# aniketntnu/WordDiffusion

Measured on AMD Instinct MI355X. Metric: denoised 64x256 word images/sec (1000-step DDPM), whole job, higher is better.
Workload: dtype bf16x3

## Files before the change

### include/wdiff_hip.h

```cpp
#ifndef WDIFF_HIP_H
#define WDIFF_HIP_H

#include <stdint.h>

#ifdef __cplusplus
extern "C" {
#endif

#define WD_OK 0
#define WD_EINVAL (-1)
#define WD_ELAUNCH (-2)
#define WD_ESTATE (-3)

#define WD_ACT_NONE 0
#define WD_ACT_SILU 1
#define WD_ACT_GEGLU 2

typedef uint16_t wd_bf16;

#define WD_MAX_KSPLIT 64

typedef struct wd_src {
    const wd_bf16* hi;
    const wd_bf16* lo;
// ... 76 lines not shown
    int32_t resid_ld;
    float* out_f32;
    int32_t out_ld;
    wd_bf16* out_hi;
    wd_bf16* out_lo;
    int32_t out_pl_ld;
    const wd_bf16* w3_hi;
    const wd_bf16* w3_lo;
    const float* b3;
    const float* resid3;
    int32_t resid3_ld;
    double* stat_part;
    int32_t stat_cpg;
    int32_t hw_out;
    int32_t npass;
} wd_ff_args;
int wd_ff_fused(const wd_ff_args* args, void* stream);
int wd_ff_supported(int c, int inner);
int wd_ff_args_bytes(void);

int wd_gemm_auto_ksplit(int m, int n, int ktot, int64_t ws_floats);
int wd_gemm_args_bytes(void);
int wd_gemm_experimental(void);

int wd_gn_nchunk(int hw);
int wd_gn_stats(const float* x, int ld, int batch, int hw, int c, int cpg, double* part, void* stream);
int wd_gn_fold_chunks(const double* part, int batch, int nchunk, int ngroups, double* out, void* stream);

int wd_gn_apply(const float* x, int ld, int batch, int hw, int c, int cpg, const double* part, int nchunk, int part_cpg,
                const float* gamma, const float* beta, float eps, int silu,
// ... 204 lines not shown
```

### worddiffusion_amd/_native.py

```python
from __future__ import annotations

import ctypes as C
import os
import re

_HERE = os.path.dirname(os.path.abspath(__file__))
LIB_PATH = os.environ.get("WDIFF_LIB") or os.path.join(_HERE, "libwdiff_hip.so")
HEADER_PATH = os.path.join(os.path.dirname(_HERE), "include", "wdiff_hip.h")

WD_OK, WD_EINVAL, WD_ELAUNCH, WD_ESTATE = 0, -1, -2, -3
ACT_NONE, ACT_SILU, ACT_GEGLU = 0, 1, 2
NCLASS = 13
CLASS_NAMES = ("gemm", "gn_stats", "gn_apply", "layernorm", "attention", "other", "gemm_other_tiles", "gemm_splitk_reduce",
               "gemm_two_per_cu", "gemm_weights_to_registers", "feed_forward_fused", "weight_gradient", "gemm_small_maps_whole_k")

_vp = C.c_void_p
_i = C.c_int
_f = C.c_float
_u64 = C.c_uint64


class WdSrc(C.Structure):
    _fields_ = [("hi", _vp), ("lo", _vp), ("gather", _vp), ("ld", C.c_int32), ("c", C.c_int32),
                ("ntaps", C.c_int32), ("hw_src", C.c_int32)]
# ... 7 lines not shown
                ("out_hi", _vp), ("out_lo", _vp), ("out_pl_ld", C.c_int32), ("tile", C.c_int32),
                ("w_layout", C.c_int32), ("slab_rows", C.c_int32), ("ksplit", C.c_int32), ("ws", _vp),
                ("ws_floats", C.c_int64), ("stat_part", _vp), ("stat_cpg", C.c_int32), ("dbg", C.c_int32),
                ("tickets", _vp), ("ntickets", C.c_int32), ("gn_gamma", _vp), ("gn_beta", _vp), ("gn_eps", C.c_float),
                ("gn_silu", C.c_int32), ("gn_cpg", C.c_int32), ("a32", _vp), ("a32_ld", C.c_int32), ("a32_part", _vp),
                ("a32_nchunk", C.c_int32), ("a32_pcpg", C.c_int32), ("a32_cpg", C.c_int32), ("a32_gamma", _vp), ("a32_beta", _vp),
                ("a32_eps", C.c_float), ("a32_silu", C.c_int32), ("ln_gamma", _vp), ("ln_beta", _vp), ("ln_eps", C.c_float),
                ("w_ngroups", C.c_int32), ("w_group_stride", C.c_int64)]


class WdFfArgs(C.Structure):
    _fields_ = [("x_hi", _vp), ("x_lo", _vp), ("x_ld", C.c_int32), ("m", C.c_int32), ("c", C.c_int32), ("inner", C.c_int32),
                ("w1_hi", _vp), ("w1_lo", _vp), ("b1", _vp), ("w2_hi", _vp), ("w2_lo", _vp), ("b2", _vp), ("resid", _vp),
                ("resid_ld", C.c_int32), ("out_f32", _vp), ("out_ld", C.c_int32), ("out_hi", _vp), ("out_lo", _vp),
                ("out_pl_ld", C.c_int32), ("w3_hi", _vp), ("w3_lo", _vp), ("b3", _vp), ("resid3", _vp), ("resid3_ld", C.c_int32),
                ("stat_part", _vp), ("stat_cpg", C.c_int32), ("hw_out", C.c_int32), ("npass", C.c_int32)]


class WdDwArgs(C.Structure):
    _fields_ = [("d_hi", _vp), ("d_lo", _vp), ("x_hi", _vp), ("x_lo", _vp), ("gather", _vp), ("grad", _vp), ("ws", _vp),
                ("ws_floats", C.c_int64), ("d_ld", C.c_int32), ("x_ld", C.c_int32), ("grad_ld", C.c_int32), ("ntaps", C.c_int32),
                ("hw_out", C.c_int32), ("hw_src", C.c_int32), ("m", C.c_int32), ("n", C.c_int32), ("c", C.c_int32),
                ("npass", C.c_int32), ("accumulate", C.c_int32), ("nslice", C.c_int32), ("dbg", C.c_int32), ("reserved", C.c_int32),
                ("stamps", _vp), ("items", _vp), ("nitems", C.c_int32), ("reserved2", C.c_int32)]


class WdDwItem(C.Structure):
    _fields_ = [("d_hi", _vp), ("d_lo", _vp), ("x_hi", _vp), ("x_lo", _vp), ("grad", _vp), ("d_ld", C.c_int32), ("x_ld", C.c_int32),
                ("grad_ld", C.c_int32), ("accumulate", C.c_int32)]


# ... 144 lines not shown
```

### worddiffusion_amd/csrc/wd_ff.hip

```cpp
#include "wd_gemm_epi.h"

namespace {

constexpr int FNT = 512;
constexpr int FBM = 64;
constexpr int FC = 320;
constexpr int FCH = 128;
constexpr int FRING = 6;
constexpr int F_MAX_INNER = 2048;
constexpr int FGRP = 30;
constexpr uint32_t F_OOB = 0x80000000u;

typedef __attribute__((ext_vector_type(4))) unsigned f_u32x4;

__device__ __forceinline__ int f_lds_off(int row, int ch) { return row * 128 + ((ch ^ ((row >> 1) & 7)) << 4); }

template <int NPASS, bool PROJ>
__global__ void __launch_bounds__(FNT, 1) wd_ff_kernel(const wd_ff_args a) {
#if defined(__HIP_DEVICE_COMPILE__)
    constexpr int NPL = (NPASS == 1) ? 1 : 2;
    constexpr int SLAB = 2 * FBM * 128;
    constexpr int A_BYTES = 5 * SLAB;
    constexpr int H_BYTES = 2 * SLAB;
    extern __shared__ __attribute__((aligned(16))) char smem[];
    char* s_a = smem;
    char* s_h = smem + A_BYTES;
    float* s_b1 = reinterpret_cast<float*>(smem + A_BYTES + 2 * H_BYTES);

    const int m0 = blockIdx.x * FBM;
    const int tid = threadIdx.x;
    const int lane = tid & 63;
    const int wave = __builtin_amdgcn_readfirstlane(tid >> 6);
    const int kh = wave >> 2, cg = wave & 3;
    const int l15 = lane & 15, lq = lane >> 4;
// ... 22 lines not shown
                ring[slot][p] = __builtin_bit_cast(bf16x8, __builtin_amdgcn_raw_buffer_load_b128(srd, lane16, so, 0));
            }
        } else if (g < 20) {
            const uint32_t so = (uint32_t)(((g >> 1) * nct1 + 2 * (j * 8 + wave) + (g & 1)) * 1024);
#pragma unroll
            for (int p = 0; p < NPL; ++p)
                ring[slot][p] = __builtin_bit_cast(bf16x8, __builtin_amdgcn_raw_buffer_load_b128(p ? srd1_lo : srd1_hi, vo, live ? so : 0u, 0));
        } else {
            const int q = (g - 20) / 5, t = (g - 20) % 5;
            const uint32_t so = (uint32_t)(((4 * j + 2 * kh + q) * (FC / 16) + 5 * cg + t) * 1024);
#pragma unroll
            for (int p = 0; p < NPL; ++p)
                ring[slot][p] = __builtin_bit_cast(bf16x8, __builtin_amdgcn_raw_buffer_load_b128(p ? srd2_lo : srd2_hi, vo, live ? so : 0u, 0));
        }
    };
#pragma unroll
    for (int g = 0; g < FRING; ++g) issue(g, g, 0);

    {
        const __amdgpu_buffer_rsrc_t sx_hi = make_srd(a.x_hi), sx_lo = make_srd(a.x_lo ? a.x_lo : a.x_hi);
        const int arow = tid >> 3, ach = tid & 7;
        const uint32_t vo = (m0 + arow < a.m) ? (uint32_t)(m0 + arow) * (uint32_t)(a.x_ld * 2) + (uint32_t)(ach * 16) : F_OOB;
        f_u32x4 v[5][NPL];
#pragma unroll
        for (int sl = 0; sl < 5; ++sl)
#pragma unroll
            for (int p = 0; p < NPL; ++p) v[sl][p] = __builtin_amdgcn_raw_buffer_load_b128(p ? sx_lo : sx_hi, vo, sl * 128, 0);
        const int dst = f_lds_off(arow, ach);
#pragma unroll
        for (int sl = 0; sl < 5; ++sl)
#pragma unroll
            for (int p = 0; p < NPL; ++p) *reinterpret_cast<f_u32x4*>(s_a + sl * SLAB + p * (FBM * 128) + dst) = v[sl][p];
        for (int i = tid; i < 2 * a.inner; i += FNT) s_b1[i] = a.b1 ? a.b1[i] : 0.0f;
    }
    __syncthreads();

    f32x4 acc2[4][5];
#pragma unroll
    for (int i = 0; i < 4; ++i)
#pragma unroll
        for (int t = 0; t < 5; ++t)
#pragma unroll
            for (int r = 0; r < 4; ++r) acc2[i][t][r] = 0.0f;

    bf16x8 xa[4][NPL];
    auto read_frags = [&](const char* slab_base, const int half) {
        const int ch = half * 4 + lq;
#pragma unroll
        for (int i = 0; i < 4; ++i) {
            const int ao = f_lds_off(i * 16 + l15, ch);
#pragma unroll
            for (int p = 0; p < NPL; ++p) xa[i][p] = *reinterpret_cast<const bf16x8*>(slab_base + p * (FBM * 128) + ao);
        }
    };
    auto mfma12 = [&](f32x4 (&acc)[4], const bf16x8 (&w)[NPL]) {
#pragma unroll
        for (int i = 0; i < 4; ++i) {
            if (NPL == 2) {
                acc[i] = __builtin_amdgcn_mfma_f32_16x16x32_bf16(xa[i][NPL - 1], w[0], acc[i], 0, 0, 0);
                acc[i] = __builtin_amdgcn_mfma_f32_16x16x32_bf16(xa[i][0], w[NPL - 1], acc[i], 0, 0, 0);
            }
            acc[i] = __builtin_amdgcn_mfma_f32_16x16x32_bf16(xa[i][0], w[0], acc[i], 0, 0, 0);
        }
    };

    for (int j = 0; j < nchunk; ++j) {
        char* hbuf = s_h + (j & 1) * H_BYTES;
        f32x4 ax[4], ag[4];
#pragma unroll
        for (int i = 0; i < 4; ++i)
#pragma unroll
            for (int r = 0; r < 4; ++r) {
                ax[i][r] = 0.0f;
                ag[i][r] = 0.0f;
            }
#pragma unroll
        for (int g = 0; g < 20; ++g) {
            if ((g & 1) == 0) read_frags(s_a + (g >> 2) * SLAB, (g >> 1) & 1);
            if (g & 1) mfma12(ag, ring[g % FRING]);
// ... 23 lines not shown
        for (int g = 20; g < FGRP; ++g) {
            const int q = (g - 20) / 5, t = (g - 20) % 5;
            if (t == 0) read_frags(hbuf + kh * SLAB, q);
            {
                f32x4 col[4] = {acc2[0][t], acc2[1][t], acc2[2][t], acc2[3][t]};
                mfma12(col, ring[g % FRING]);
#pragma unroll
                for (int i = 0; i < 4; ++i) acc2[i][t] = col[i];
            }
            if (g + FRING < FGRP) issue(g % FRING, g + FRING, j);
            else issue(g % FRING, g + FRING - FGRP, j + 1);
            __builtin_amdgcn_sched_barrier(0);
        }
    }

    constexpr int LDE = FC + 4;
    float* ep = reinterpret_cast<float*>(smem);
    __syncthreads();
    for (int hh = 0; hh < 2; ++hh) {
        if (kh == hh) {
#pragma unroll
            for (int i = 0; i < 4; ++i)
#pragma unroll
                for (int t = 0; t < 5; ++t)
#pragma unroll
                    for (int r = 0; r < 4; ++r) {
                        float* pe = ep + (i * 16 + 4 * lq + r) * LDE + cg * 80 + t * 16 + l15;
                        *pe = (hh == 0) ? acc2[i][t][r] : *pe + acc2[i][t][r];
                    }
        }
        __syncthreads();
    }
    wd_gemm_args e = {};
    e.m = a.m;
    e.n = FC;
    e.hw_out = a.hw_out > 0 ? a.hw_out : 1;
    e.act = WD_ACT_NONE;
    e.out_f32 = a.out_f32;
    e.out_ld = a.out_ld;
    e.out_hi = a.out_hi;
    e.out_lo = a.out_lo;
    e.out_pl_ld = a.out_pl_ld;
    e.ksplit = 1;
    e.stat_part = a.stat_part;
    e.stat_cpg = a.stat_cpg;
    if constexpr (!PROJ) {
        e.bias = a.b2;
        e.resid = a.resid;
        e.resid_ld = a.resid_ld;
        wd_epilogue_from_image<FBM, FC, FNT>(e, ep, m0, 0, tid);
    } else {
        constexpr int ROWB = LDE * 4;
        {
            float4 v[10];
#pragma unroll
            for (int it = 0; it < 10; ++it) {
                const int idx = it * 64 + lane, row = wave * 8 + idx / 80, c = (idx % 80) * 4;
                const int m = m0 + row;
                float4 x = *reinterpret_cast<const float4*>(ep + row * LDE + c);
                if (a.b2) {
                    const float4 q = *reinterpret_cast<const float4*>(a.b2 + c);
                    x.x += q.x; x.y += q.y; x.z += q.z; x.w += q.w;
                }
                if (a.resid && m < a.m) {
                    const float4 q = *reinterpret_cast<const float4*>(a.resid + (long)m * a.resid_ld + c);
                    x.x += q.x; x.y += q.y; x.z += q.z; x.w += q.w;
                }
                v[it] = x;
            }
            asm volatile("s_waitcnt lgkmcnt(0)" ::: "memory");
            __builtin_amdgcn_sched_barrier(0);
#pragma unroll
            for (int it = 0; it < 10; ++it) {
                const int idx = it * 64 + lane, row = wave * 8 + idx / 80, c = (idx % 80) * 4;
                uint2 hh, ll;
                wd_split4(v[it], hh, ll);
                char* rowp = reinterpret_cast<char*>(ep) + row * ROWB;
                *reinterpret_cast<uint2*>(rowp + c * 2) = hh;
                if (NPL == 2) *reinterpret_cast<uint2*>(rowp + 640 + c * 2) = ll;
            }
// ... 21 lines not shown
                f32x4 col[4] = {acc2[0][t], acc2[1][t], acc2[2][t], acc2[3][t]};
                mfma12(col, ring[g % FRING]);
#pragma unroll
                for (int i = 0; i < 4; ++i) acc2[i][t] = col[i];
            }
            if (g + FRING < 25) {
                const int g2 = g + FRING;
                const uint32_t so3 = (uint32_t)(((2 * (g2 / 5) + kh) * (FC / 16) + 5 * cg + g2 % 5) * 1024);
#pragma unroll
                for (int p = 0; p < NPL; ++p)
                    ring[g % FRING][p] = __builtin_bit_cast(bf16x8, __builtin_amdgcn_raw_buffer_load_b128(p ? srd3_lo : srd3_hi, lane16, so3, 0));
            }
            __builtin_amdgcn_sched_barrier(0);
        }
        __syncthreads();
        for (int hh = 0; hh < 2; ++hh) {
            if (kh == hh) {
#pragma unroll
                for (int i = 0; i < 4; ++i)
#pragma unroll
                    for (int t = 0; t < 5; ++t)
#pragma unroll
                        for (int r = 0; r < 4; ++r) {
                            float* pe = ep + (i * 16 + 4 * lq + r) * LDE + cg * 80 + t * 16 + l15;
                            *pe = (hh == 0) ? acc2[i][t][r] : *pe + acc2[i][t][r];
                        }
            }
            __syncthreads();
        }
        e.bias = a.b3;
        e.resid = a.resid3;
        e.resid_ld = a.resid3_ld;
        wd_epilogue_from_image<FBM, FC, FNT>(e, ep, m0, 0, tid);
    }
#endif
}

template <int NPASS, bool PROJ>
int launch_ff(const wd_ff_args& a, hipStream_t st) {
    constexpr int max_smem = 5 * 2 * FBM * 128 + 2 * 2 * 2 * FBM * 128 + 2 * F_MAX_INNER * 4;
    constexpr int red_smem = FBM * (FC + 4) * 4 + WD_STAT_SCRATCH;
    static_assert(max_smem <= 160 * 1024 && red_smem <= max_smem, "LDS budget");
    const int loop_smem = max_smem - 2 * (F_MAX_INNER - a.inner) * 4;
    const int smem = loop_smem > red_smem ? loop_smem : red_smem;
    static bool attr_done = false;
    if (!attr_done) {
        if (hipFuncSetAttribute(reinterpret_cast<const void*>(&wd_ff_kernel<NPASS, PROJ>), hipFuncAttributeMaxDynamicSharedMemorySize,
                                max_smem) != hipSuccess)
            return WD_ELAUNCH;
        attr_done = true;
    }
    const int nb = (a.m + FBM - 1) / FBM;
    const double fl = 2.0 * (double)a.m * (3.0 * (double)a.inner * FC + (PROJ ? (double)FC * FC : 0.0));
    WdLaunchScope scope(WD_CLS_FF, st, fl);
    hipLaunchKernelGGL((wd_ff_kernel<NPASS, PROJ>), dim3(nb), dim3(FNT), smem, st, a);
    return wd_check_launch();
}

}

extern "C" int wd_ff_args_bytes(void) { return (int)sizeof(wd_ff_args); }

extern "C" int wd_ff_supported(int c, int inner) { return (c == FC && inner > 0 && inner % FCH == 0 && inner <= F_MAX_INNER) ? 1 : 0; }

extern "C" int wd_ff_fused(const wd_ff_args* pa, void* stream) {
    if (!pa) return WD_EINVAL;
    const wd_ff_args& a = *pa;
    if (!wd_ff_supported(a.c, a.inner) || a.m <= 0 || (a.npass != 1 && a.npass != 3)) return WD_EINVAL;
    if (!a.x_hi || !a.w1_hi || !a.w2_hi || (a.npass == 3 && (!a.x_lo || !a.w1_lo || !a.w2_lo))) return WD_EINVAL;
    if (!a.out_f32 && !a.out_hi) return WD_EINVAL;
    if (a.x_ld % 8 || a.x_ld < a.c) return WD_EINVAL;
    if ((a.out_ld | a.resid_ld | a.out_pl_ld) & 3) return WD_EINVAL;
    if (a.resid && a.resid_ld <= 0) return WD_EINVAL;
    if ((long)a.m * a.x_ld * 2 >= 0x7FFFFFF0L || (long)2 * a.inner * a.c * 2 >= 0x7FFFFFF0L) return WD_EINVAL;
    const bool proj = a.w3_hi != nullptr;
    if (proj && ((a.npass == 3 && !a.w3_lo) || (a.resid3 && (a.resid3_ld <= 0 || (a.resid3_ld & 3))))) return WD_EINVAL;
    if (a.stat_part && (a.stat_cpg <= 0 || FC % a.stat_cpg || a.hw_out <= 0 || !(a.hw_out % FBM == 0 || FBM % a.hw_out == 0) ||
                        (FBM > a.hw_out && FBM / a.hw_out > WD_STAT_MAXNS)))
        return WD_EINVAL;
    hipStream_t st = reinterpret_cast<hipStream_t>(stream);
    if (proj) return a.npass == 3 ? launch_ff<3, true>(a, st) : launch_ff<1, true>(a, st);
    return a.npass == 3 ? launch_ff<3, false>(a, st) : launch_ff<1, false>(a, st);
}
```

### worddiffusion_amd/engine.py

```python
from __future__ import annotations

import ctypes as C
import math
import os
from typing import Dict, List, Optional, Tuple

import numpy as np
import torch

from . import _native as N
from .layers import (DownsampleParams, ResBlockParams, SpatialTransformerParams, UpsampleParams)


def conv_gather_table(h: int, w: int, mode: str) -> Tuple[np.ndarray, int, int]:
    if mode == "same":
        ho, wo = h, w
    elif mode == "down":
        ho, wo = (h + 2 - 3) // 2 + 1, (w + 2 - 3) // 2 + 1
    elif mode == "up":
        ho, wo = 2 * h, 2 * w
    else:
        raise ValueError(mode)
    yy, xx = np.meshgrid(np.arange(ho), np.arange(wo), indexing="ij")
    tab = np.full((9, ho * wo), -1, dtype=np.int32)
# ... 272 lines not shown
        self.use_up_phases = os.environ.get("WDIFF_UPSAMPLE_PHASES", "1") != "0"
        self._derived: Dict[str, tuple] = {}
        self.use_smallmap = os.environ.get("WDIFF_GEMM_SMALLMAP", "1") != "0"
        self.fuse_ff = os.environ.get("WDIFF_FUSE_FF", "1") != "0"
        self.fuse_proj = os.environ.get("WDIFF_FUSE_PROJ", "1") != "0"
        self.fuse_ln = os.environ.get("WDIFF_FUSE_LN", "1") != "0"
        self.fuse_gn_in = int(os.environ.get("WDIFF_FUSE_GN_IN", "1"))
        self.use_slab = os.environ.get("WDIFF_SLAB", "0") != "0"
        self.fuse_stats = os.environ.get("WDIFF_FUSE_STATS", "1") != "0"
        self.fuse_xattn = os.environ.get("WDIFF_FUSE_XATTN", "1") != "0"
        self.use_conv3 = os.environ.get("WDIFF_CONV3", "0") != "0"
        if (self.use_slab or self.use_conv3) and not self.lib.wd_gemm_experimental():
            raise N.NativeError("WDIFF_SLAB / WDIFF_CONV3 need a library built with WDIFF_EXPERIMENTAL=1 "
                                "(python -m worddiffusion_amd.build --force)")
        self.fuse_xattn_pair = os.environ.get("WDIFF_FUSE_XATTN_PAIR", "1") != "0"
        self.fuse_out = os.environ.get("WDIFF_FUSE_OUT", "1") != "0"
        self.pack_kv = os.environ.get("WDIFF_PACK_KV", "1") != "0"
        self.fuse_gn2 = os.environ.get("WDIFF_FUSE_GN2", "1") != "0"
        self.fuse_gn = os.environ.get("WDIFF_FUSE_GN", "1") != "0"
        self.fuse_split = os.environ.get("WDIFF_FUSE_SPLIT", "1") != "0"
        self._plans: Dict[tuple, Plan] = {}
        self._tabs: Dict[tuple, torch.Tensor] = {}
        self._tab_np: Dict[int, np.ndarray] = {}
        self._same_w: Dict[int, int] = {}
        self._down_w: Dict[int, int] = {}
        self._ws = None
        self.device = None

    def set_precision(self, mode: str):
        npass = {"bf16x3": 3, "fp32": 3, "bf16": 1}[mode]
# ... 544 lines not shown
        ops.append((self.lib.wd_attention,
                    (q, ldq, k, ldk, v, ldv, B, heads, nq, nk, d, float(scale), _ptr(out_f32),
                     out_pl[0].data_ptr() if out_pl is not None else None,
                     out_pl[1].data_ptr() if (out_pl is not None and self.npass == 3) else None,
                     out_pl.shape[2] if out_pl is not None else out_f32.shape[-1],
                     nq if out_rows is None else out_rows, out_row0), what))

    def _transformer(self, P, name, mod: SpatialTransformerParams, x: Act) -> Act:
        ops = P.step
        B = self._B
        h, w, c = x.h, x.w, x.c
        hw, M = h * w, B * h * w
        heads, d = mod.heads, mod.d_head
        inner = heads * d
        L = self._ctx_len
        tok = self._f32(P, M, inner)
        n1_pre = None
        ln1 = None
        if self.variant == "phosc" and self._ln_in_producer(M, inner):
            n1_pre, ln1 = self._planes(P, M, inner), f"{name}.tb0.norm1"
        if self._gn_in_consumer(P, ops, name + ".gn", [x], False, M, hw, inner):
            self._gemm(ops, name + ".proj_in", [self._src32(x, hw_src=hw)], name + ".pi.w", M, hw, bias=self._w[name + ".pi.b"],
                       out_f32=tok, out_ld=inner, a32=(x, name + ".gn", 1e-6, False), out_pl=n1_pre, ln=ln1)
        else:
            g, _ = self._gn(P, ops, name + ".gn", [x], name + ".gn", 1e-6, False)
            self._gemm(ops, name + ".proj_in", [self._src(g, c)], name + ".pi.w", M, hw, bias=self._w[name + ".pi.b"],
                       out_f32=tok, out_ld=inner, out_pl=n1_pre, ln=ln1)
        xpl = None
        fuse = self.fuse_xattn and bool(self.lib.wd_xattn_supported(inner, heads, L))

# ... 117 lines not shown
                    return Act(out, c, h, w, fa._stats, prod=fa)
                self._ff_fused(ops, p, n3, tok2, M, inner, ffi, None if last else tok, xpl)
            else:
                ffh = self._planes(P, M, ffi)
                self._gemm(ops, p + ".ff1", [self._src(n3, inner)], p + ".ff1.w", M, hw, bias=self._w[p + ".ff1.b"],
                           act=N.ACT_GEGLU, out_pl=ffh, tile=geglu_tile(ffi))
                self._gemm(ops, p + ".ff2", [self._src(ffh, ffi)], p + ".ff2.w", M, hw, bias=self._w[p + ".ff2.b"],
                           resid=tok2.data_ptr(), resid_ld=inner, out_f32=None if last else tok, out_ld=inner,
                           out_pl=xpl)
        out = self._f32(P, M, c)
        gg = self._gemm(ops, name + ".proj_out", [self._src(xpl, inner)], name + ".po.w", M, hw,
                        bias=self._w[name + ".po.b"], resid=x.t.data_ptr(), resid_ld=c, out_f32=out, out_ld=c,
                        want_stats=True)
        return Act(out, c, h, w, gg._stats, prod=gg)

    def _wfrag(self, wname):
        if wname not in self._wf:
            self._wf[wname] = torch.empty_like(self._w[wname])
            self._pack_wf(wname, self._wf[wname], torch.cuda.current_stream(self.device).cuda_stream)
            self._pack = None
        return self._wf[wname]

    def _ff_fused(self, ops, p, n3, resid, M, inner, ffi, out_f32, out_pl, proj=None):
        a = N.WdFfArgs()
        lo_ok = self.npass == 3
        a.x_hi, a.x_lo, a.x_ld = n3[0].data_ptr(), (n3[1].data_ptr() if lo_ok else None), n3.shape[2]
        a.m, a.c, a.inner = M, inner, ffi
        w1, w2 = self._wfrag(p + ".ff1f.w"), self._wfrag(p + ".ff2.w")
        a.w1_hi, a.w1_lo, a.b1 = w1[0].data_ptr(), w1[1].data_ptr(), self._w[p + ".ff1f.b"].data_ptr()
        a.w2_hi, a.w2_lo, a.b2 = w2[0].data_ptr(), w2[1].data_ptr(), self._w[p + ".ff2.b"].data_ptr()
        a.resid, a.resid_ld = resid.data_ptr(), inner
        if out_f32 is not None:
            a.out_f32, a.out_ld = out_f32.data_ptr(), inner
        if out_pl is not None:
            a.out_hi, a.out_lo, a.out_pl_ld = out_pl[0].data_ptr(), (out_pl[1].data_ptr() if lo_ok else None), out_pl.shape[2]
        a.hw_out, a.npass = 1, self.npass
        stats = None
        if proj is not None:
            wname, b3, x_in, hw = proj
            w3 = self._wfrag(wname)
            a.w3_hi, a.w3_lo, a.b3 = w3[0].data_ptr(), w3[1].data_ptr(), b3.data_ptr()
            a.resid3, a.resid3_ld = x_in.data_ptr(), inner
            if self.fuse_stats and inner % 32 == 0 and hw % 64 == 0:
                nchunk = hw // 64
                part = torch.zeros((M // hw, nchunk, 32, 2), dtype=torch.float64, device=self.device)
                self._cur_plan.keep.append(part)
                a.stat_part, a.stat_cpg, a.hw_out = part.data_ptr(), inner // 32, hw
                stats = (part, nchunk, inner // 32)
        self._cur_plan.keep.append(a)
        ops.append((self.lib.wd_ff_fused, (C.byref(a),), p + (".ff + proj_out (fused)" if proj is not None else ".ff (fused)")))
        a._stats = stats
        return a

    def plan(self, B: int, H: int, W: int, ctx_len: int, phosc_len: int, film_steps: int = 0) -> Plan:
        key = (B, H, W, ctx_len, phosc_len, self.npass, film_steps)
        if key in self._plans:
            self._plans[key] = self._plans.pop(key)
            return self._plans[key]
        while len(self._plans) >= max(1, PLAN_CACHE_SIZE):
            self._plans.pop(next(iter(self._plans)))
        m = self.model
        lib = self.lib
        if ctx_len + phosc_len == 0:
            raise NotImplementedError("context=None: every reference script conditions on the word (unet.py:1605)")
        P = Plan()
# ... 210 lines not shown
```

Baseline: 33.42.

## Fuse entire spatial transformer block into one feed-forward kernel launch

Extends the fused feed-forward kernel with a front section that applies group norm from partial stats, runs proj_in, then two cross-attention passes (using precomputed folded query/output matrices), layer norms, and finally feed-forward plus proj_out. This is all in one launch per 64-row tile, enabled by default for 320-channel single-block transformers. It removes several kernel launches and the HBM round trips of intermediate activations between them. The cost is much higher per-block register and LDS pressure, and a narrow eligibility condition.

```diff
diff --git a/include/wdiff_hip.h b/include/wdiff_hip.h
--- a/include/wdiff_hip.h
+++ b/include/wdiff_hip.h
@@ -114,6 +114,30 @@
     int32_t stat_cpg;
     int32_t hw_out;
     int32_t npass;
+    const float* x_in;
+    int32_t x_in_ld;
+    int32_t hw;
+    const double* gn_part;
+    int32_t gn_nchunk, gn_pcpg, gn_cpg;
+    float gn_eps;
+    const float* gn_gamma;
+    const float* gn_beta;
+    const wd_bf16* pi_hi;
+    const wd_bf16* pi_lo;
+    const float* pi_b;
+    const float* ln2_gamma;
+    const float* ln2_beta;
+    const wd_bf16* mq_a;
+    const wd_bf16* mot_a;
+    const float* xb_a;
+    const wd_bf16* mq_b;
+    const wd_bf16* mot_b;
+    const float* xb_b;
+    const float* ln3_gamma;
+    const float* ln3_beta;
+    float ln_eps;
+    int32_t heads, L;
+    float* tok2;
 } wd_ff_args;
 int wd_ff_fused(const wd_ff_args* args, void* stream);
 int wd_ff_supported(int c, int inner);
diff --git a/worddiffusion_amd/_native.py b/worddiffusion_amd/_native.py
--- a/worddiffusion_amd/_native.py
+++ b/worddiffusion_amd/_native.py
@@ -45,7 +45,12 @@
                 ("w1_hi", _vp), ("w1_lo", _vp), ("b1", _vp), ("w2_hi", _vp), ("w2_lo", _vp), ("b2", _vp), ("resid", _vp),
                 ("resid_ld", C.c_int32), ("out_f32", _vp), ("out_ld", C.c_int32), ("out_hi", _vp), ("out_lo", _vp),
                 ("out_pl_ld", C.c_int32), ("w3_hi", _vp), ("w3_lo", _vp), ("b3", _vp), ("resid3", _vp), ("resid3_ld", C.c_int32),
-                ("stat_part", _vp), ("stat_cpg", C.c_int32), ("hw_out", C.c_int32), ("npass", C.c_int32)]
+                ("stat_part", _vp), ("stat_cpg", C.c_int32), ("hw_out", C.c_int32), ("npass", C.c_int32),
+                ("x_in", _vp), ("x_in_ld", C.c_int32), ("hw", C.c_int32), ("gn_part", _vp), ("gn_nchunk", C.c_int32),
+                ("gn_pcpg", C.c_int32), ("gn_cpg", C.c_int32), ("gn_eps", C.c_float), ("gn_gamma", _vp), ("gn_beta", _vp),
+                ("pi_hi", _vp), ("pi_lo", _vp), ("pi_b", _vp), ("ln2_gamma", _vp), ("ln2_beta", _vp), ("mq_a", _vp), ("mot_a", _vp),
+                ("xb_a", _vp), ("mq_b", _vp), ("mot_b", _vp), ("xb_b", _vp), ("ln3_gamma", _vp), ("ln3_beta", _vp),
+                ("ln_eps", C.c_float), ("heads", C.c_int32), ("L", C.c_int32), ("tok2", _vp)]
 
 
 class WdDwArgs(C.Structure):
diff --git a/worddiffusion_amd/csrc/wd_ff.hip b/worddiffusion_amd/csrc/wd_ff.hip
--- a/worddiffusion_amd/csrc/wd_ff.hip
+++ b/worddiffusion_amd/csrc/wd_ff.hip
@@ -15,9 +15,10 @@
 
 __device__ __forceinline__ int f_lds_off(int row, int ch) { return row * 128 + ((ch ^ ((row >> 1) & 7)) << 4); }
 
-template <int NPASS, bool PROJ>
+template <int NPASS, bool PROJ, bool FRONT>
 __global__ void __launch_bounds__(FNT, 1) wd_ff_kernel(const wd_ff_args a) {
 #if defined(__HIP_DEVICE_COMPILE__)
+    static_assert(!FRONT || (NPASS == 3 && PROJ), "the transformer front needs split-bf16 operands and the proj_out tail");
     constexpr int NPL = (NPASS == 1) ? 1 : 2;
     constexpr int SLAB = 2 * FBM * 128;
     constexpr int A_BYTES = 5 * SLAB;
@@ -70,6 +71,307 @@
                 ring[slot][p] = __builtin_bit_cast(bf16x8, __builtin_amdgcn_raw_buffer_load_b128(p ? srd2_lo : srd2_hi, vo, live ? so : 0u, 0));
         }
     };
+    f32x4 acc2[4][5];
+    bf16x8 xa[4][NPL];
+    auto read_frags = [&](const char* slab_base, const int half) {
+        const int ch = half * 4 + lq;
+#pragma unroll
+        for (int i = 0; i < 4; ++i) {
+            const int ao = f_lds_off(i * 16 + l15, ch);
+#pragma unroll
+            for (int p = 0; p < NPL; ++p) xa[i][p] = *reinterpret_cast<const bf16x8*>(slab_base + p * (FBM * 128) + ao);
+        }
+    };
+    auto mfma12 = [&](f32x4 (&acc)[4], const bf16x8 (&w)[NPL]) {
+#pragma unroll
+        for (int i = 0; i < 4; ++i) {
+            if (NPL == 2) {
+                acc[i] = __builtin_amdgcn_mfma_f32_16x16x32_bf16(xa[i][NPL - 1], w[0], acc[i], 0, 0, 0);
+                acc[i] = __builtin_amdgcn_mfma_f32_16x16x32_bf16(xa[i][0], w[NPL - 1], acc[i], 0, 0, 0);
+            }
+            acc[i] = __builtin_amdgcn_mfma_f32_16x16x32_bf16(xa[i][0], w[0], acc[i], 0, 0, 0);
+        }
+    };
+    constexpr int LDE = FC + 4;
+    float* ep = reinterpret_cast<float*>(smem);
+    auto ksum_to_image = [&]() {
+        for (int hh = 0; hh < 2; ++hh) {
+            if (kh == hh) {
+#pragma unroll
+                for (int i = 0; i < 4; ++i)
+#pragma unroll
+                    for (int t = 0; t < 5; ++t)
+#pragma unroll
+                        for (int r = 0; r < 4; ++r) {
+                            float* pe = ep + (i * 16 + 4 * lq + r) * LDE + cg * 80 + t * 16 + l15;
+                            *pe = (hh == 0) ? acc2[i][t][r] : *pe + acc2[i][t][r];
+                        }
+            }
+            __syncthreads();
+        }
+    };
+
+    if constexpr (FRONT) {
+        constexpr int SP = 65, PP = 72, KS32 = FC / 32;
+        const int b = m0 / a.hw;
+        const int HJ = a.heads * a.L;
+        char* fr = s_h + 4096;
+        float* s_aff = reinterpret_cast<float*>(fr);
+        float* sS = reinterpret_cast<float*>(fr);
+        wd_bf16* sP = reinterpret_cast<wd_bf16*>(fr + FBM * SP * 4);
+        {
+            const int ngp = FC / a.gn_pcpg, ratio = a.gn_cpg / a.gn_pcpg;
+            for (int c = tid; c < FC; c += FNT) {
+                const int g = c / a.gn_cpg;
+                double su = 0.0, sq = 0.0;
+                for (int k = 0; k < ratio; ++k)
+                    for (int ck = 0; ck < a.gn_nchunk; ++ck) {
+                        const double* pp = a.gn_part + (((long)b * a.gn_nchunk + ck) * ngp + g * ratio + k) * 2;
+                        su += pp[0];
+                        sq += pp[1];
+                    }
+                const double n = (double)a.hw * a.gn_cpg;
+                const double mu = su / n;
+                double var = sq / n - mu * mu;
+                if (var < 0.0) var = 0.0;
+                const float rstd = (float)(1.0 / sqrt(var + (double)a.gn_eps));
+                const float sc = rstd * a.gn_gamma[c];
+                s_aff[2 * c] = sc;
+                s_aff[2 * c + 1] = a.gn_beta[c] - (float)mu * sc;
+            }
+            for (int e = tid; e < FBM * PP; e += FNT) reinterpret_cast<uint32_t*>(sP)[e] = 0u;
+        }
+        const int arow = tid >> 3, ach = tid & 7;
+        float4 xv[5][2];
+        {
+            const float* xrow = a.x_in + (long)(m0 + arow) * a.x_in_ld + ach * 8;
+#pragma unroll
+            for (int sl = 0; sl < 5; ++sl) {
+                xv[sl][0] = *reinterpret_cast<const float4*>(xrow + sl * 64);
+                xv[sl][1] = *reinterpret_cast<const float4*>(xrow + sl * 64 + 4);
+            }
+        }
+        const __amdgpu_buffer_rsrc_t srdp_hi = make_srd(a.pi_hi), srdp_lo = make_srd(a.pi_lo);
+        auto issue_pi = [&](const int slot, const int g) {
+            const uint32_t so = (uint32_t)(((2 * (g / 5) + kh) * (FC / 16) + 5 * cg + g % 5) * 1024);
+#pragma unroll
+            for (int p = 0; p < NPL; ++p)
+                ring[slot][p] = __builtin_bit_cast(bf16x8, __builtin_amdgcn_raw_buffer_load_b128(p ? srdp_lo : srdp_hi, lane16, so, 0));
+        };
+#pragma unroll
+        for (int g = 0; g < FRING; ++g) issue_pi(g, g);
+        __syncthreads();
+#pragma unroll
+        for (int sl = 0; sl < 5; ++sl) {
+            const float4* tab = reinterpret_cast<const float4*>(s_aff + 2 * (sl * 64 + ach * 8));
+            const float4 t0 = tab[0], t1 = tab[1], t2 = tab[2], t3 = tab[3];
+            const float4 x0 = xv[sl][0], x1 = xv[sl][1];
+            float4 y0, y1;
+            y0.x = x0.x * t0.x + t0.y; y0.y = x0.y * t0.z + t0.w; y0.z = x0.z * t1.x + t1.y; y0.w = x0.w * t1.z + t1.w;
+            y1.x = x1.x * t2.x + t2.y; y1.y = x1.y * t2.z + t2.w; y1.z = x1.z * t3.x + t3.y; y1.w = x1.w * t3.z + t3.w;
+            uint2 h0, l0, h1, l1;
+            wd_split4(y0, h0, l0);
+            wd_split4(y1, h1, l1);
+            char* dst = s_a + sl * SLAB + f_lds_off(arow, ach);
+            *reinterpret_cast<f_u32x4*>(dst) = f_u32x4{h0.x, h0.y, h1.x, h1.y};
+            *reinterpret_cast<f_u32x4*>(dst + FBM * 128) = f_u32x4{l0.x, l0.y, l1.x, l1.y};
+        }
+        __syncthreads();
+#pragma unroll
+        for (int i = 0; i < 4; ++i)
+#pragma unroll
+            for (int t = 0; t < 5; ++t)
+#pragma unroll
+                for (int r = 0; r < 4; ++r) acc2[i][t][r] = 0.0f;
+#pragma unroll
+        for (int g = 0; g < 25; ++g) {
+            const int q = g / 5, t = g % 5;
+            if (t == 0) read_frags(s_a + q * SLAB, kh);
+            {
+                f32x4 col[4] = {acc2[0][t], acc2[1][t], acc2[2][t], acc2[3][t]};
+                mfma12(col, ring[g % FRING]);
+#pragma unroll
+                for (int i = 0; i < 4; ++i) acc2[i][t] = col[i];
+            }
+            if (g + FRING < 25) issue_pi(g % FRING, g + FRING);
+            __builtin_amdgcn_sched_barrier(0);
+        }
+        __syncthreads();
+        ksum_to_image();
+        float4 xr[2][5];
+#pragma unroll
+        for (int pp = 0; pp < 2; ++pp)
+#pragma unroll
+            for (int i = 0; i < 5; ++i) {
+                const int n = (l15 + 16 * i) * 4, row = wave * 8 + pp * 4 + lq;
+                const float4 v = *reinterpret_cast<const float4*>(ep + row * LDE + n);
+                const float4 bx = *reinterpret_cast<const float4*>(a.pi_b + n);
+                xr[pp][i] = make_float4(v.x + bx.x, v.y + bx.y, v.z + bx.z, v.w + bx.w);
+            }
+        __syncthreads();
+        auto ln_rows = [&](const float* gamma, const float* beta) {
+#pragma unroll
+            for (int pp = 0; pp < 2; ++pp) {
+                const int row = wave * 8 + pp * 4 + lq;
+                float s = 0.f;
+#pragma unroll
+                for (int i = 0; i < 5; ++i) s += (xr[pp][i].x + xr[pp][i].y) + (xr[pp][i].z + xr[pp][i].w);
+                const float mean = wd_row16_sum(s) / (float)FC;
+                float q = 0.f;
+#pragma unroll
+                for (int i = 0; i < 5; ++i) {
+                    const float a0 = xr[pp][i].x - mean, a1 = xr[pp][i].y - mean, a2 = xr[pp][i].z - mean, a3 = xr[pp][i].w - mean;
+                    q += (a0 * a0 + a1 * a1) + (a2 * a2 + a3 * a3);
+                }
+                const float rstd = 1.0f / sqrtf(wd_row16_sum(q) / (float)FC + a.ln_eps);
+#pragma unroll
+                for (int i = 0; i < 5; ++i) {
+                    const int n = (l15 + 16 * i) * 4;
+                    const float4 ga = *reinterpret_cast<const float4*>(gamma + n);
+                    const float4 be = *reinterpret_cast<const float4*>(beta + n);
+                    const float4 x = xr[pp][i];
+                    float4 o;
+                    o.x = (x.x - mean) * rstd * ga.x + be.x; o.y = (x.y - mean) * rstd * ga.y + be.y;
+                    o.z = (x.z - mean) * rstd * ga.z + be.z; o.w = (x.w - mean) * rstd * ga.w + be.w;
+                    uint2 hi, lo;
+                    wd_split4(o, hi, lo);
+                    char* d = s_a + (n >> 6) * SLAB + f_lds_off(row, (n & 63) >> 3) + (n & 7) * 2;
+                    *reinterpret_cast<uint2*>(d) = hi;
+                    *reinterpret_cast<uint2*>(d + FBM * 128) = lo;
+                }
+            }
+        };
+        const int ht = wave & 3, rp = wave >> 2;
+        const long pq = 64L * FC;
+#pragma unroll
+        for (int ps = 0; ps < 2; ++ps) {
+            const wd_bf16* mq = ps == 0 ? a.mq_a : a.mq_b;
+            const wd_bf16* mot = ps == 0 ? a.mot_a : a.mot_b;
+            const float* xb = ps == 0 ? a.xb_a : a.xb_b;
+            ln_rows(a.ln2_gamma, a.ln2_beta);
+            __builtin_amdgcn_sched_barrier(0);
+            bf16x8 bh[KS32], bl[KS32];
+            {
+                const __amdgpu_buffer_rsrc_t rq = __builtin_amdgcn_make_buffer_rsrc(const_cast<wd_bf16*>(mq + (long)b * 2 * pq), 0,
+                                                                                    (int)(2 * pq * 2), 0x00020000);
+                const uint32_t vo = ht * 16 + l15 < HJ ? lane16 : F_OOB;
+#pragma unroll
+                for (int ks = 0; ks < KS32; ++ks) {
+                    bh[ks] = __builtin_bit_cast(bf16x8, __builtin_amdgcn_raw_buffer_load_b128(rq, vo, (uint32_t)((ht * KS32 + ks) << 10), 0));
+                    bl[ks] = __builtin_bit_cast(bf16x8, __builtin_amdgcn_raw_buffer_load_b128(rq, vo, (uint32_t)(((ht * KS32 + ks) << 10) + pq * 2), 0));
+                }
+            }
+            __syncthreads();
+            if (ht * 16 < HJ) {
+                f32x4 a_lh[2], a_hl[2], a_hh[2];
+#pragma unroll
+                for (int ri = 0; ri < 2; ++ri)
+#pragma unroll
+                    for (int r = 0; r < 4; ++r) a_lh[ri][r] = a_hl[ri][r] = a_hh[ri][r] = 0.f;
+#pragma unroll
+                for (int ks = 0; ks < KS32; ++ks)
+#pragma unroll
+                    for (int ri = 0; ri < 2; ++ri) {
+                        const char* ap = s_a + (ks >> 1) * SLAB + f_lds_off((2 * rp + ri) * 16 + l15, (ks & 1) * 4 + lq);
+                        const bf16x8 ah = *reinterpret_cast<const bf16x8*>(ap);
+                        const bf16x8 al = *reinterpret_cast<const bf16x8*>(ap + FBM * 128);
+                        a_lh[ri] = __builtin_amdgcn_mfma_f32_16x16x32_bf16(al, bh[ks], a_lh[ri], 0, 0, 0);
+                        a_hl[ri] = __builtin_amdgcn_mfma_f32_16x16x32_bf16(ah, bl[ks], a_hl[ri], 0, 0, 0);
+                        a_hh[ri] = __builtin_amdgcn_mfma_f32_16x16x32_bf16(ah, bh[ks], a_hh[ri], 0, 0, 0);
+                    }
+#pragma unroll
+                for (int ri = 0; ri < 2; ++ri)
+#pragma unroll
+                    for (int r = 0; r < 4; ++r)
+                        sS[((2 * rp + ri) * 16 + 4 * lq + r) * SP + ht * 16 + l15] = (a_lh[ri][r] + a_hl[ri][r]) + a_hh[ri][r];
+            }
+            __builtin_amdgcn_sched_barrier(0);
+            bf16x8 mh[2][5], ml[2][5];
+            {
+                const __amdgpu_buffer_rsrc_t rm = __builtin_amdgcn_make_buffer_rsrc(const_cast<wd_bf16*>(mot + (long)b * 2 * pq), 0,
+                                                                                    (int)(2 * pq * 2), 0x00020000);
+#pragma unroll
+                for (int ks = 0; ks < 2; ++ks) {
+                    const uint32_t vo = ks * 32 + lq * 8 < HJ ? lane16 : F_OOB;
+#pragma unroll
+                    for (int t = 0; t < 5; ++t) {
+                        const uint32_t so = (uint32_t)((((5 * cg + t) * 2 + ks) << 10));
+                        mh[ks][t] = __builtin_bit_cast(bf16x8, __builtin_amdgcn_raw_buffer_load_b128(rm, vo, so, 0));
+                        ml[ks][t] = __builtin_bit_cast(bf16x8, __builtin_amdgcn_raw_buffer_load_b128(rm, vo, so + (uint32_t)(pq * 2), 0));
+                    }
+                }
+            }
+            __syncthreads();
+            for (int idx = tid; idx < FBM * a.heads; idx += FNT) {
+                const int t = idx / a.heads, h = idx - t * a.heads;
+                const float* pr = sS + t * SP + h * a.L;
+                wd_bf16* ph = sP + t * PP + h * a.L;
+                float mx = -3.4e38f;
+                for (int j = 0; j < a.L; ++j) mx = fmaxf(mx, pr[j]);
+                float sum = 0.f;
+                for (int j = 0; j < a.L; ++j) sum += __expf(pr[j] - mx);
+                const float inv = __fdividef(1.f, sum);
+                for (int j = 0; j < a.L; ++j) {
+                    uint32_t hi, lo;
+                    wd_split1(__expf(pr[j] - mx) * inv, hi, lo);
+                    ph[j] = (wd_bf16)hi;
+                    ph[FBM * PP + j] = (wd_bf16)lo;
+                }
+            }
+            __syncthreads();
+            {
+                f32x4 o[2][5];
+#pragma unroll
+                for (int ri = 0; ri < 2; ++ri)
+#pragma unroll
+                    for (int t = 0; t < 5; ++t)
+#pragma unroll
+                        for (int r = 0; r < 4; ++r) o[ri][t][r] = 0.f;
+#pragma unroll
+                for (int ks = 0; ks < 2; ++ks)
+#pragma unroll
+                    for (int ri = 0; ri < 2; ++ri) {
+                        const wd_bf16* ap = sP + ((2 * rp + ri) * 16 + l15) * PP + lq * 8 + ks * 32;
+                        const bf16x8 ah = *reinterpret_cast<const bf16x8*>(ap);
+                        const bf16x8 al = *reinterpret_cast<const bf16x8*>(ap + FBM * PP);
+#pragma unroll
+                        for (int t = 0; t < 5; ++t) o[ri][t] = __builtin_amdgcn_mfma_f32_16x16x32_bf16(al, mh[ks][t], o[ri][t], 0, 0, 0);
+#pragma unroll
+                        for (int t = 0; t < 5; ++t) o[ri][t] = __builtin_amdgcn_mfma_f32_16x16x32_bf16(ah, ml[ks][t], o[ri][t], 0, 0, 0);
+#pragma unroll
+                        for (int t = 0; t < 5; ++t) o[ri][t] = __builtin_amdgcn_mfma_f32_16x16x32_bf16(ah, mh[ks][t], o[ri][t], 0, 0, 0);
+                    }
+#pragma unroll
+                for (int ri = 0; ri < 2; ++ri)
+#pragma unroll
+                    for (int t = 0; t < 5; ++t)
+#pragma unroll
+                        for (int r = 0; r < 4; ++r) ep[((2 * rp + ri) * 16 + 4 * lq + r) * LDE + (5 * cg + t) * 16 + l15] = o[ri][t][r];
+            }
+            __syncthreads();
+#pragma unroll
+            for (int pp = 0; pp < 2; ++pp)
+#pragma unroll
+                for (int i = 0; i < 5; ++i) {
+                    const int n = (l15 + 16 * i) * 4, row = wave * 8 + pp * 4 + lq;
+                    const float4 bi = *reinterpret_cast<const float4*>(xb + n);
+                    const float4 at = *reinterpret_cast<const float4*>(ep + row * LDE + n);
+                    const float4 x = xr[pp][i];
+                    xr[pp][i] = make_float4(at.x + bi.x + x.x, at.y + bi.y + x.y, at.z + bi.z + x.z, at.w + bi.w + x.w);
+                }
+            __syncthreads();
+        }
+#pragma unroll
+        for (int pp = 0; pp < 2; ++pp)
+#pragma unroll
+            for (int i = 0; i < 5; ++i)
+                *reinterpret_cast<float4*>(a.tok2 + (long)(m0 + wave * 8 + pp * 4 + lq) * FC + (l15 + 16 * i) * 4) = xr[pp][i];
+        ln_rows(a.ln3_gamma, a.ln3_beta);
+        for (int i = tid; i < 2 * a.inner; i += FNT) s_b1[i] = a.b1 ? a.b1[i] : 0.0f;
+        __builtin_amdgcn_sched_barrier(0);
+#pragma unroll
+        for (int g = 0; g < FRING; ++g) issue(g, g, 0);
+    } else {
 #pragma unroll
     for (int g = 0; g < FRING; ++g) issue(g, g, 0);
 
@@ -89,36 +391,15 @@
             for (int p = 0; p < NPL; ++p) *reinterpret_cast<f_u32x4*>(s_a + sl * SLAB + p * (FBM * 128) + dst) = v[sl][p];
         for (int i = tid; i < 2 * a.inner; i += FNT) s_b1[i] = a.b1 ? a.b1[i] : 0.0f;
     }
+    }
     __syncthreads();
 
-    f32x4 acc2[4][5];
 #pragma unroll
     for (int i = 0; i < 4; ++i)
 #pragma unroll
         for (int t = 0; t < 5; ++t)
 #pragma unroll
             for (int r = 0; r < 4; ++r) acc2[i][t][r] = 0.0f;
-
-    bf16x8 xa[4][NPL];
-    auto read_frags = [&](const char* slab_base, const int half) {
-        const int ch = half * 4 + lq;
-#pragma unroll
-        for (int i = 0; i < 4; ++i) {
-            const int ao = f_lds_off(i * 16 + l15, ch);
-#pragma unroll
-            for (int p = 0; p < NPL; ++p) xa[i][p] = *reinterpret_cast<const bf16x8*>(slab_base + p * (FBM * 128) + ao);
-        }
-    };
-    auto mfma12 = [&](f32x4 (&acc)[4], const bf16x8 (&w)[NPL]) {
-#pragma unroll
-        for (int i = 0; i < 4; ++i) {
-            if (NPL == 2) {
-                acc[i] = __builtin_amdgcn_mfma_f32_16x16x32_bf16(xa[i][NPL - 1], w[0], acc[i], 0, 0, 0);
-                acc[i] = __builtin_amdgcn_mfma_f32_16x16x32_bf16(xa[i][0], w[NPL - 1], acc[i], 0, 0, 0);
-            }
-            acc[i] = __builtin_amdgcn_mfma_f32_16x16x32_bf16(xa[i][0], w[0], acc[i], 0, 0, 0);
-        }
-    };
 
     for (int j = 0; j < nchunk; ++j) {
         char* hbuf = s_h + (j & 1) * H_BYTES;
@@ -172,23 +453,8 @@
         }
     }
 
-    constexpr int LDE = FC + 4;
-    float* ep = reinterpret_cast<float*>(smem);
     __syncthreads();
-    for (int hh = 0; hh < 2; ++hh) {
-        if (kh == hh) {
-#pragma unroll
-            for (int i = 0; i < 4; ++i)
-#pragma unroll
-                for (int t = 0; t < 5; ++t)
-#pragma unroll
-                    for (int r = 0; r < 4; ++r) {
-                        float* pe = ep + (i * 16 + 4 * lq + r) * LDE + cg * 80 + t * 16 + l15;
-                        *pe = (hh == 0) ? acc2[i][t][r] : *pe + acc2[i][t][r];
-                    }
-        }
-        __syncthreads();
-    }
+    ksum_to_image();
     wd_gemm_args e = {};
     e.m = a.m;
     e.n = FC;
@@ -209,6 +475,9 @@
         wd_epilogue_from_image<FBM, FC, FNT>(e, ep, m0, 0, tid);
     } else {
         constexpr int ROWB = LDE * 4;
+        const float* resid = FRONT ? a.tok2 : a.resid;
+        const int resid_ld = FRONT ? FC : a.resid_ld;
+        if (FRONT) asm volatile("s_waitcnt vmcnt(0)" ::: "memory");
         {
             float4 v[10];
 #pragma unroll
@@ -220,8 +489,8 @@
                     const float4 q = *reinterpret_cast<const float4*>(a.b2 + c);
                     x.x += q.x; x.y += q.y; x.z += q.z; x.w += q.w;
                 }
-                if (a.resid && m < a.m) {
-                    const float4 q = *reinterpret_cast<const float4*>(a.resid + (long)m * a.resid_ld + c);
+                if (resid && m < a.m) {
+                    const float4 q = *reinterpret_cast<const float4*>(resid + (long)m * resid_ld + c);
                     x.x += q.x; x.y += q.y; x.z += q.z; x.w += q.w;
                 }
                 v[it] = x;
@@ -273,20 +542,7 @@
             __builtin_amdgcn_sched_barrier(0);
         }
         __syncthreads();
-        for (int hh = 0; hh < 2; ++hh) {
-            if (kh == hh) {
-#pragma unroll
-                for (int i = 0; i < 4; ++i)
-#pragma unroll
-                    for (int t = 0; t < 5; ++t)
-#pragma unroll
-                        for (int r = 0; r < 4; ++r) {
-                            float* pe = ep + (i * 16 + 4 * lq + r) * LDE + cg * 80 + t * 16 + l15;
-                            *pe = (hh == 0) ? acc2[i][t][r] : *pe + acc2[i][t][r];
-                        }
-            }
-            __syncthreads();
-        }
+        ksum_to_image();
         e.bias = a.b3;
         e.resid = a.resid3;
         e.resid_ld = a.resid3_ld;
@@ -295,7 +551,7 @@
 #endif
 }
 
-template <int NPASS, bool PROJ>
+template <int NPASS, bool PROJ, bool FRONT = false>
 int launch_ff(const wd_ff_args& a, hipStream_t st) {
     constexpr int max_smem = 5 * 2 * FBM * 128 + 2 * 2 * 2 * FBM * 128 + 2 * F_MAX_INNER * 4;
     constexpr int red_smem = FBM * (FC + 4) * 4 + WD_STAT_SCRATCH;
@@ -304,15 +560,16 @@
     const int smem = loop_smem > red_smem ? loop_smem : red_smem;
     static bool attr_done = false;
     if (!attr_done) {
-        if (hipFuncSetAttribute(reinterpret_cast<const void*>(&wd_ff_kernel<NPASS, PROJ>), hipFuncAttributeMaxDynamicSharedMemorySize,
+        if (hipFuncSetAttribute(reinterpret_cast<const void*>(&wd_ff_kernel<NPASS, PROJ, FRONT>), hipFuncAttributeMaxDynamicSharedMemorySize,
                                 max_smem) != hipSuccess)
             return WD_ELAUNCH;
         attr_done = true;
     }
     const int nb = (a.m + FBM - 1) / FBM;
-    const double fl = 2.0 * (double)a.m * (3.0 * (double)a.inner * FC + (PROJ ? (double)FC * FC : 0.0));
+    const double fl = 2.0 * (double)a.m * (3.0 * (double)a.inner * FC + (PROJ ? (double)FC * FC : 0.0) +
+                                           (FRONT ? (double)FC * FC + 4.0 * a.heads * a.L * FC : 0.0));
     WdLaunchScope scope(WD_CLS_FF, st, fl);
-    hipLaunchKernelGGL((wd_ff_kernel<NPASS, PROJ>), dim3(nb), dim3(FNT), smem, st, a);
+    hipLaunchKernelGGL((wd_ff_kernel<NPASS, PROJ, FRONT>), dim3(nb), dim3(FNT), smem, st, a);
     return wd_check_launch();
 }
 
@@ -326,9 +583,10 @@
     if (!pa) return WD_EINVAL;
     const wd_ff_args& a = *pa;
     if (!wd_ff_supported(a.c, a.inner) || a.m <= 0 || (a.npass != 1 && a.npass != 3)) return WD_EINVAL;
-    if (!a.x_hi || !a.w1_hi || !a.w2_hi || (a.npass == 3 && (!a.x_lo || !a.w1_lo || !a.w2_lo))) return WD_EINVAL;
+    const bool front = a.x_in != nullptr;
+    if (!a.w1_hi || !a.w2_hi || (a.npass == 3 && (!a.w1_lo || !a.w2_lo))) return WD_EINVAL;
+    if (!front && (!a.x_hi || (a.npass == 3 && !a.x_lo) || a.x_ld % 8 || a.x_ld < a.c)) return WD_EINVAL;
     if (!a.out_f32 && !a.out_hi) return WD_EINVAL;
-    if (a.x_ld % 8 || a.x_ld < a.c) return WD_EINVAL;
     if ((a.out_ld | a.resid_ld | a.out_pl_ld) & 3) return WD_EINVAL;
     if (a.resid && a.resid_ld <= 0) return WD_EINVAL;
     if ((long)a.m * a.x_ld * 2 >= 0x7FFFFFF0L || (long)2 * a.inner * a.c * 2 >= 0x7FFFFFF0L) return WD_EINVAL;
@@ -337,7 +595,16 @@
     if (a.stat_part && (a.stat_cpg <= 0 || FC % a.stat_cpg || a.hw_out <= 0 || !(a.hw_out % FBM == 0 || FBM % a.hw_out == 0) ||
                         (FBM > a.hw_out && FBM / a.hw_out > WD_STAT_MAXNS)))
         return WD_EINVAL;
+    if (front) {
+        if (a.npass != 3 || !proj || a.x_in_ld < a.c || a.x_in_ld % 4 || a.hw <= 0 || a.hw % FBM || a.m % a.hw) return WD_EINVAL;
+        if (!a.gn_part || a.gn_nchunk <= 0 || a.gn_pcpg <= 0 || a.gn_cpg <= 0 || a.gn_cpg % a.gn_pcpg || FC % a.gn_cpg ||
+            !a.gn_gamma || !a.gn_beta)
+            return WD_EINVAL;
+        if (!a.pi_hi || !a.pi_lo || !a.pi_b || !a.ln2_gamma || !a.ln2_beta || !a.ln3_gamma || !a.ln3_beta || !a.tok2) return WD_EINVAL;
+        if (!a.mq_a || !a.mot_a || !a.xb_a || !a.mq_b || !a.mot_b || !a.xb_b || !wd_xattn_supported(a.c, a.heads, a.L)) return WD_EINVAL;
+    }
     hipStream_t st = reinterpret_cast<hipStream_t>(stream);
+    if (front) return launch_ff<3, true, true>(a, st);
     if (proj) return a.npass == 3 ? launch_ff<3, true>(a, st) : launch_ff<1, true>(a, st);
     return a.npass == 3 ? launch_ff<3, false>(a, st) : launch_ff<1, false>(a, st);
 }
diff --git a/worddiffusion_amd/engine.py b/worddiffusion_amd/engine.py
--- a/worddiffusion_amd/engine.py
+++ b/worddiffusion_amd/engine.py
@@ -310,6 +310,7 @@
             raise N.NativeError("WDIFF_SLAB / WDIFF_CONV3 need a library built with WDIFF_EXPERIMENTAL=1 "
                                 "(python -m worddiffusion_amd.build --force)")
         self.fuse_xattn_pair = os.environ.get("WDIFF_FUSE_XATTN_PAIR", "1") != "0"
+        self.fuse_st = os.environ.get("WDIFF_FUSE_ST", "1") != "0"
         self.fuse_out = os.environ.get("WDIFF_FUSE_OUT", "1") != "0"
         self.pack_kv = os.environ.get("WDIFF_PACK_KV", "1") != "0"
         self.fuse_gn2 = os.environ.get("WDIFF_FUSE_GN2", "1") != "0"
@@ -884,6 +885,12 @@
         heads, d = mod.heads, mod.d_head
         inner = heads * d
         L = self._ctx_len
+        if (self.fuse_st and self.variant != "phosc" and len(mod.transformer_blocks) == 1 and inner == c == 320 and
+                self.npass == 3 and self.fuse_xattn and self.fuse_xattn_pair and self.fuse_ff and self.fuse_proj and
+                bool(self.lib.wd_xattn_supported(inner, heads, L)) and (M + 63) // 64 >= 192 and hw % 64 == 0 and
+                (name + ".tb0.ff1f.w") in self._w and
+                self._gn_in_consumer(P, ops, name + ".gn", [x], False, M, hw, inner)):
+            return self._transformer_fused(P, name, mod, x)
         tok = self._f32(P, M, inner)
         n1_pre = None
         ln1 = None
@@ -1031,6 +1038,41 @@
                         want_stats=True)
         return Act(out, c, h, w, gg._stats, prod=gg)
 
+    def _transformer_fused(self, P, name, mod: SpatialTransformerParams, x: Act) -> Act:
+        B, M, hw, c = self._B, self._B * x.h * x.w, x.h * x.w, x.c
+        heads, d, L = mod.heads, mod.d_head, self._ctx_len
+        p = name + ".tb0"
+        folds = []
+        for tag in ("a1", "a2"):
+            ko = self.kv_off[f"{p}.{tag}"]
+            mq = self._f32(P, B, heads * L, c)
+            mo = self._f32(P, B, heads * L, c)
+            mq_pl = torch.zeros((B, 2, 64, c), dtype=torch.bfloat16, device=self.device)
+            mot_pl = torch.zeros((B, 2, c, 64), dtype=torch.bfloat16, device=self.device)
+            P.keep += [mq_pl, mot_pl]
+            P.cond.append((self.lib.wd_xattn_fold,
+                           (self._kv.data_ptr() + 4 * ko, self.kv_total, self._kv.data_ptr() + 4 * (ko + c), self.kv_total, B,
+                            heads, L, d, float(d ** -0.5), self._w[f"{p}.{tag}.q.f32"].data_ptr(),
+                            self._w[f"{p}.{tag}.o.f32"].data_ptr(), c, mq.data_ptr(), mo.data_ptr(), mq_pl.data_ptr(),
+                            mot_pl.data_ptr()), f"{p}.{tag}:fold"))
+            folds.append((mq_pl, mot_pl))
+        tok2 = self._f32(P, M, c)
+        out = self._f32(P, M, c)
+        part, nchunk, pc = x.stats
+        pw = self._wfrag(name + ".pi.w")
+        front = dict(x_in=x.t.data_ptr(), x_in_ld=c, hw=hw, gn_part=part.data_ptr(), gn_nchunk=nchunk, gn_pcpg=pc, gn_cpg=c // 32,
+                     gn_eps=1e-6, gn_gamma=self._w[name + ".gn.g"].data_ptr(), gn_beta=self._w[name + ".gn.b"].data_ptr(),
+                     pi_hi=pw[0].data_ptr(), pi_lo=pw[1].data_ptr(), pi_b=self._w[name + ".pi.b"].data_ptr(),
+                     ln2_gamma=self._w[p + ".norm2.g"].data_ptr(), ln2_beta=self._w[p + ".norm2.b"].data_ptr(),
+                     mq_a=folds[0][0].data_ptr(), mot_a=folds[0][1].data_ptr(), xb_a=self._w[p + ".a1.o.b"].data_ptr(),
+                     mq_b=folds[1][0].data_ptr(), mot_b=folds[1][1].data_ptr(), xb_b=self._w[p + ".a2.o.b"].data_ptr(),
+                     ln3_gamma=self._w[p + ".norm3.g"].data_ptr(), ln3_beta=self._w[p + ".norm3.b"].data_ptr(), ln_eps=1e-5,
+                     heads=heads, L=L, tok2=tok2.data_ptr())
+        ffi = mod.transformer_blocks[0].ff.net[2].in_features
+        fa = self._ff_fused(P.step, p, None, tok2, M, c, ffi, out, None, proj=(name + ".po.w", self._w[name + ".po.b"], x.t, hw),
+                            front=front)
+        return Act(out, c, x.h, x.w, fa._stats, prod=fa)
+
     def _wfrag(self, wname):
         if wname not in self._wf:
             self._wf[wname] = torch.empty_like(self._w[wname])
@@ -1038,10 +1080,14 @@
             self._pack = None
         return self._wf[wname]
 
-    def _ff_fused(self, ops, p, n3, resid, M, inner, ffi, out_f32, out_pl, proj=None):
+    def _ff_fused(self, ops, p, n3, resid, M, inner, ffi, out_f32, out_pl, proj=None, front=None):
         a = N.WdFfArgs()
         lo_ok = self.npass == 3
-        a.x_hi, a.x_lo, a.x_ld = n3[0].data_ptr(), (n3[1].data_ptr() if lo_ok else None), n3.shape[2]
+        if front is None:
+            a.x_hi, a.x_lo, a.x_ld = n3[0].data_ptr(), (n3[1].data_ptr() if lo_ok else None), n3.shape[2]
+        else:
+            for k, v in front.items():
+                setattr(a, k, v)
         a.m, a.c, a.inner = M, inner, ffi
         w1, w2 = self._wfrag(p + ".ff1f.w"), self._wfrag(p + ".ff2.w")
         a.w1_hi, a.w1_lo, a.b1 = w1[0].data_ptr(), w1[1].data_ptr(), self._w[p + ".ff1f.b"].data_ptr()
@@ -1065,7 +1111,8 @@
                 a.stat_part, a.stat_cpg, a.hw_out = part.data_ptr(), inner // 32, hw
                 stats = (part, nchunk, inner // 32)
         self._cur_plan.keep.append(a)
-        ops.append((self.lib.wd_ff_fused, (C.byref(a),), p + (".ff + proj_out (fused)" if proj is not None else ".ff (fused)")))
+        what = ".ff (fused)" if proj is None else ".ff + proj_out (fused)" if front is None else ": gn + proj_in + a1 + a2 + ff + proj_out (fused)"
+        ops.append((self.lib.wd_ff_fused, (C.byref(a),), p + what))
         a._stats = stats
         return a
 
```

Result: faster. 34.27, median of 6 (+2.5%).
